# sbelharbi/feature-vs-text-compound-emotion

Measured on AMD Instinct MI355X. Metric: training clips/sec (32-frame tri-modal clip), higher is better.
Workload: dtype bf16x3 (split hi/lo bf16 operands, 3 MFMAs per product, fp32 accumulate; <= 2^-15 relative per product)

## Files before the change

### feature_vs_text_compound_emotion_amd/csrc/conv_b3.h

```cpp
#pragma once
#include "conv_common.h"

namespace cer {

typedef __bf16 bf16x8 __attribute__((ext_vector_type(8)));
typedef unsigned int u32x4 __attribute__((ext_vector_type(4)));
typedef __attribute__((address_space(3))) void *lds_ptr_t;

__device__ __forceinline__ bf16x8 as_bf16x8(const u32x4 v) { return __builtin_bit_cast(bf16x8, v); }


typedef float f32x4 __attribute__((ext_vector_type(4)));
__device__ __forceinline__ int swz16(int q) { return (0x78 >> (2 * q)) & 3; }

int conv_b3_patch_launch(int tile, const ConvArgs &a, hipStream_t st);
bool conv_b3_patch_ok(const ConvArgs &a);
bool conv_b3_win_ok(const ConvArgs &a);
int conv_b3_s2d_launch(int tile, const ConvArgs &a, hipStream_t st);
bool conv_b3_s2d_ok(const ConvArgs &a);

}
```

### feature_vs_text_compound_emotion_amd/csrc/conv_b3.hip

```cpp
#include "conv_b3.h"

namespace cer {

template <int BM, int BN, int WP, int WC, int NW = 4, int STAGES = 2>
__global__ __launch_bounds__(NW * 64, NW == 4 ? 2 : 1) void conv_b3_dma16_kernel(ConvArgs p) {
    static_assert(WP * WC == NW && BM % (16 * NW) == 0 && BN % (16 * NW) == 0, "1-KiB pieces are dealt round-robin to the waves");
    constexpr int BKT = 32, ROWB = BKT * 2;
    constexpr int XP = BM / (16 * NW), WQ = BN / (16 * NW);
    constexpr int PX = BM * ROWB, PW = BN * ROWB;
    constexpr int BUF = 2 * PX + 2 * PW;
    constexpr int NDMA = 2 * XP + 2 * WQ;
    static_assert(STAGES == 2 || STAGES == 3, "ring depth");
    constexpr int TP = BM / (16 * WP), TC = BN / (16 * WC);
    constexpr unsigned OOB = 0x80000000u;
    extern __shared__ __attribute__((aligned(16))) uint16_t smem_b3[];
    unsigned char *smem = reinterpret_cast<unsigned char *>(smem_b3);

    const int tid = threadIdx.x, lane = tid & 63;
    const int wave = __builtin_amdgcn_readfirstlane(tid >> 6);
    const int wp = wave % WP, wc = wave / WP;
    const int kg = lane >> 4, l15 = lane & 15;

    const int nwg = p.tiles_m * p.tiles_n;
    int bid = blockIdx.x;
// ... 247 lines not shown
                    const int m = m0 + (wp * TP + b) * 16 + l15;
                    const float v = (m < p.M) ? acc[a][b][r] : 0.f;
                    s1 += v;
                    s2 += v * v;
                });
#pragma unroll
                for (int o = 8; o > 0; o >>= 1) {
                    s1 += __shfl_xor(s1, o);
                    s2 += __shfl_xor(s2, o);
                }
                if (l15 == 0) {
                    const int ci = (wc * TC + a) * 16 + 4 * kg + r;
                    red[(wp * 2 + 0) * BN + ci] = s1;
                    red[(wp * 2 + 1) * BN + ci] = s2;
                }
            });
        });
        __syncthreads();
        if (tid < BN && c0 + tid < p.Cout) {
            float s1 = 0.f, s2 = 0.f;
#pragma unroll
            for (int w = 0; w < WP; ++w) {
                s1 += red[(w * 2 + 0) * BN + tid];
                s2 += red[(w * 2 + 1) * BN + tid];
            }
            p.stats[((size_t)tile_m * 2 + 0) * p.Cout + c0 + tid] = s1;
            p.stats[((size_t)tile_m * 2 + 1) * p.Cout + c0 + tid] = s2;
        }
    }
}

__global__ void split_bf16_kernel(const float4 *__restrict__ x, const float *__restrict__ scale,
                                  const float *__restrict__ shift, ushort4 *__restrict__ hi, ushort4 *__restrict__ lo,
                                  size_t n4, int C4) {
    size_t i = (size_t)blockIdx.x * blockDim.x + threadIdx.x;
    if (i >= n4) return;
    float4 v = x[i];
    if (scale) {
        const int c = (int)(i % C4) * 4;
        const float4 s = *reinterpret_cast<const float4 *>(scale + c), t = *reinterpret_cast<const float4 *>(shift + c);
        v = make_float4(v.x * s.x + t.x, v.y * s.y + t.y, v.z * s.z + t.z, v.w * s.w + t.w);
    }
    ushort4 h, l;
    split_bf16(v.x, h.x, l.x); split_bf16(v.y, h.y, l.y);
    split_bf16(v.z, h.z, l.z); split_bf16(v.w, h.w, l.w);
    hi[i] = h;
    lo[i] = l;
}

template <int BM, int BN, int WP, int WC, int NW = 4, int STAGES = 2>
static int launch_b3_dma16(const ConvArgs &a, hipStream_t st) {
    if ((long long)BN * a.Kpad * 2 >= (1ll << 31))
        return cer_set_error(CER_ERR_UNSUPPORTED, "conv2d (bf16x3, LDS-DMA): weight panel exceeds 31-bit offsets");
    const size_t lds = (size_t)STAGES * (2 * BM + 2 * BN) * 64;
    auto k = conv_b3_dma16_kernel<BM, BN, WP, WC, NW, STAGES>;
    if (lds > 64 * 1024) CER_HIP_CHECK(hipFuncSetAttribute((const void *)k, hipFuncAttributeMaxDynamicSharedMemorySize, (int)lds));
    CER_LAUNCH(k, dim3(a.tiles_m * a.tiles_n, 1, a.split_k), dim3(NW * 64), lds, st, a);
    CER_HIP_CHECK(hipGetLastError());
    return CER_OK;
}

static bool b3_patch_geometry(const cer_conv_desc *d) {
    return d->KH == 3 && d->KW == 3 && d->stride == 1 && d->dil_h == 1 && d->dil_w == 1 && d->pad_t == 1 && d->pad_l == 1 &&
           d->Ho == d->H && d->Wo == d->W && (d->H & 15) == 0 && (d->W & 15) == 0 && (d->Cin & 31) == 0 && d->split_k <= 1;
}

static bool b3_win_geometry(const cer_conv_desc *d) {
    return d->KH == 3 && d->KW == 3 && d->stride == 1 && d->dil_h == 1 && d->dil_w == 1 && d->pad_t == 1 && d->pad_l == 1 &&
           d->Ho == d->H && d->Wo == d->W && d->H >= 2 && d->W >= 2 && d->W <= 86 && (d->Cin & 31) == 0 && d->split_k <= 1;
}

int conv_b3_tile_dims(const cer_conv_desc *d, int &bm, int &bn, int &bk) {
    int tile = d->tile;
    const long long M = (long long)d->N * d->Ho * d->Wo;
    const int Cout = d->Cout;
    if (d->x_s2d) {
        if (tile == 0) tile = Cout > 64 ? 52 : 51;
        else if (tile != 51 && tile != 52) return 0;
    } else if (tile == 51 || tile == 52) {
        return 0;
    }
    if (tile == 0) {
        const long long t128 = (M + 127) / 128 * ((Cout + 127) / 128), t256 = (M + 255) / 256;
        if (b3_patch_geometry(d) && Cout <= 64 && t256 >= 512) tile = 59;
        else if (b3_patch_geometry(d) && Cout >= 128 && t256 * ((Cout + 127) / 128) >= 512) tile = 58;
        else if (b3_win_geometry(d) && t256 >= 64) tile = Cout > 64 ? 56 : 53;
        else if (Cout <= 64) tile = t256 >= 512 ? 48 : 42;
        else if (t128 >= 512) tile = 41;
        else tile = Cout >= 128 ? 44 : 45;
    }
    bk = 32;
    switch (tile) {
        case 41: bm = 128; bn = 128; break;
        case 42: bm = 128; bn = 64; break;
        case 44: bm = 64; bn = 128; break;
        case 45: bm = 64; bn = 64; break;
        case 48: bm = 256; bn = 64; break;
        case 59: bm = 256; bn = 64; break;
        case 58: bm = 256; bn = 128; break;
        case 53: bm = 256; bn = 64; break;
        case 56: bm = 256; bn = 128; break;
        case 51: bm = 256; bn = 64; break;
        case 52: bm = 256; bn = 128; break;
        default: return 0;
    }
    return tile;
}

int conv_b3_launch(int tile, const ConvArgs &a, hipStream_t st) {
    switch (tile) {
        case 41: return launch_b3_dma16<128, 128, 2, 2>(a, st);
        case 42: return launch_b3_dma16<128, 64, 2, 2>(a, st);
        case 44: return launch_b3_dma16<64, 128, 1, 4>(a, st);
        case 45: return launch_b3_dma16<64, 64, 2, 2>(a, st);
        case 48: return launch_b3_dma16<256, 64, 4, 1>(a, st);
        case 53: case 56: case 58: case 59: return conv_b3_patch_launch(tile, a, st);
        case 51: case 52: return conv_b3_s2d_launch(tile, a, st);
        default: return cer_set_error(CER_ERR_INVALID_ARG, "conv2d (bf16x3): unknown tile id");
    }
}

}

using namespace cer;

extern "C" int cer_conv2d_b3_tile(const cer_conv_desc *d) {
    if (!d || d->N <= 0 || d->Ho <= 0 || d->Wo <= 0 || d->Cout <= 0) return 0;
    int bm, bn, bk;
    return conv_b3_tile_dims(d, bm, bn, bk);
}

extern "C" int cer_split_bf16(const float *x, const float *scale, const float *shift, int C, uint16_t *hi, uint16_t *lo,
                              size_t n, void *stream) {
    if (!x || !hi || !lo || n == 0 || (n & 3)) return cer_set_error(CER_ERR_INVALID_ARG, "split_bf16: n must be a positive multiple of 4");
    if ((scale == nullptr) != (shift == nullptr) || (scale && (C <= 0 || (C & 3) || n % C)))
        return cer_set_error(CER_ERR_INVALID_ARG, "split_bf16: the per-channel affine needs scale, shift and C % 4 == 0 dividing n");
    CER_LAUNCH(split_bf16_kernel, dim3(cer_blocks(n / 4, 256)), dim3(256), 0, (hipStream_t)stream, (const float4 *)x, scale,
               shift, (ushort4 *)hi, (ushort4 *)lo, n / 4, scale ? C / 4 : 1);
    CER_HIP_CHECK(hipGetLastError());
    return CER_OK;
}
```

### feature_vs_text_compound_emotion_amd/csrc/conv_b3_patch.hip

```cpp
#include "conv_b3.h"

namespace cer {

constexpr unsigned long long B3_PATCH_F_TABLE = 0xaaa00a00ull;
__device__ __forceinline__ int b3_patch_f(int wx) { return (int)((B3_PATCH_F_TABLE >> (2 * wx)) & 3ull); }

struct B3PatchGeo { FastDiv tiles_n, pxn, pyn; };

template <int BN, int WP, int WC, bool SINGLE>
__global__ __launch_bounds__(WP * WC * 64, 2) void conv_b3_patch_kernel(ConvArgs p, B3PatchGeo geo) {
    constexpr int NW = WP * WC, NT = NW * 64;
    constexpr int PH = 16, PWD = 16, WW = 18, WROWS = 18 * 18;
    constexpr int XPP = (WROWS + 15) / 16;
    constexpr int XPW = (XPP + NW - 1) / NW;
    constexpr int XPL = XPP * 1024, XBYTES = 2 * XPL;
    constexpr int WPL = BN * 64, WSLICE = 2 * WPL;
    constexpr int WPIECES = 2 * BN / 16;
    static_assert(WPIECES % NW == 0, "weight-slice pieces are dealt round-robin to the waves");
    constexpr int WQ = WPIECES / NW;
    constexpr int TP = PH / WP, TC = BN / (16 * WC);
    static_assert(PH % WP == 0 && (SINGLE || XPW <= 9) && TP >= 2 && TC % 2 == 0, "geometry");
    static_assert(SINGLE ? WC == 1 : (WP == 4 && WC == 2 && (BN / 16) % 4 == 0), "ping-pong: waves w and w + 4 share a SIMD and split the couts");
    constexpr int WOFF = (SINGLE ? 1 : 2) * XBYTES, SINK = WOFF + 3 * WSLICE;
    constexpr unsigned OOB = 0x80000000u;
    extern __shared__ __attribute__((aligned(16))) uint16_t smem_b3p[];
    unsigned char *smem = reinterpret_cast<unsigned char *>(smem_b3p);

    const int tid = threadIdx.x, lane = tid & 63;
    const int wave = __builtin_amdgcn_readfirstlane(tid >> 6);
    const int wp = wave % WP, wc = wave / WP;
    const int kg = lane >> 4, l15 = lane & 15;

    const int nwg = p.tiles_m * p.tiles_n;
    int bid = blockIdx.x;
    {
        const int q = nwg >> 3, r = nwg & 7, xcd = bid & 7, idx = bid >> 3;
        bid = (xcd < r ? xcd * (q + 1) : r * (q + 1) + (xcd - r) * q) + idx;
    }
    const int patch = (int)fdiv((unsigned)bid, geo.tiles_n), tile_n = bid - patch * p.tiles_n;
    const int prw = (int)fdiv((unsigned)patch, geo.pxn), px = patch - prw * (int)geo.pxn.d;
    const int n = (int)fdiv((unsigned)prw, geo.pyn), py = prw - n * (int)geo.pyn.d;
    const int c0 = tile_n * BN;
    const int cin_steps = p.cin_steps;

    const int prow = lane >> 2, slot = lane & 3;
    unsigned x_off[XPW];
    bool x_real[XPW];
    {
        const int iy0 = py * PH - 1, ix0 = px * PWD - 1, pitch = p.x_ld * 2;
#pragma unroll
        for (int i = 0; i < XPW; ++i) {
            const int q = wave + NW * i;
            const int row = q * 16 + prow;
            const int wy = row / WW, wx = row - wy * WW;
            const int iy = iy0 + wy, ix = ix0 + wx;
            const bool inb = q < XPP && row < WROWS && (unsigned)iy < (unsigned)p.H && (unsigned)ix < (unsigned)p.W;
            x_real[i] = q < XPP;
            x_off[i] = inb ? (unsigned)((iy * p.W + ix) * pitch) + (unsigned)((slot ^ b3_patch_f(wx)) << 4) : OOB;
        }
    }
    unsigned w_off[WQ];
    int w_plane[WQ], w_dst[WQ];
#pragma unroll
    for (int i = 0; i < WQ; ++i) {
        const int j = SINGLE ? wave + NW * i : (wave & 3) + 4 * i;
        constexpr int PPL = SINGLE ? BN / 16 : BN / 32;
        w_plane[i] = j / PPL;
        const int pc = (SINGLE ? 0 : (wave >> 2) * PPL) + j % PPL;
        const int row = pc * 16 + prow;
        const int grow = row / (TC * 16) * (TC * 16) + epi_cout_of_row(row % (TC * 16));
        w_dst[i] = w_plane[i] * WPL + pc * 1024;
        w_off[i] = c0 + grow < p.Cout ? (unsigned)(grow * p.Kpad * 2) + (unsigned)((slot ^ swz16((row >> 2) & 3)) << 4) : OOB;
    }
    const size_t img = (size_t)n * p.H * p.W * p.x_ld * 2;
    const char *xh = reinterpret_cast<const char *>(p.x_hi) + img, *xl = reinterpret_cast<const char *>(p.x_lo) + img;
    const size_t wpan = (size_t)c0 * p.Kpad * 2;
    const char *wh = reinterpret_cast<const char *>(p.w_hi) + wpan, *wl = reinterpret_cast<const char *>(p.w_lo) + wpan;

    auto issue_x = [&](int i, int cc) {
        const bool real = x_real[i] && cc < cin_steps;
        const __amdgpu_buffer_rsrc_t rh = __builtin_amdgcn_make_buffer_rsrc(const_cast<char *>(xh) + (size_t)cc * 64, 0, (int)OOB, 0x00020000);
        const __amdgpu_buffer_rsrc_t rl = __builtin_amdgcn_make_buffer_rsrc(const_cast<char *>(xl) + (size_t)cc * 64, 0, (int)OOB, 0x00020000);
        unsigned char *dst = real ? smem + (SINGLE ? 0 : (cc & 1) * XBYTES) + (wave + NW * i) * 1024 : smem + SINK;
        const int vo = (int)(real ? x_off[i] : OOB);
        __builtin_amdgcn_raw_ptr_buffer_load_lds(rh, (lds_ptr_t)dst, 16, vo, 0, 0, 0);
        __builtin_amdgcn_raw_ptr_buffer_load_lds(rl, (lds_ptr_t)(real ? dst + XPL : dst), 16, vo, 0, 0, 0);
    };
    auto issue_w = [&](int cc, int tap, int ring) {
        const bool real = cc < cin_steps;
        const size_t koff = ((size_t)tap * p.Cin + (size_t)cc * 32) * 2;
// ... 591 lines not shown
```

### feature_vs_text_compound_emotion_amd/csrc/conv_igemm.hip

```cpp
#include <hip/hip_runtime.h>
#include <stdint.h>

#include "cer_internal.h"
#include "conv_common.h"

namespace cer {

template <int BM, int BN, int WP, int WC, bool VEC, int VAR, int BKT>
__global__ __launch_bounds__(WP * WC * 64, 3) void conv_igemm_kernel(ConvArgs p) {
    constexpr int NT = WP * WC * 64;
    constexpr int CH = BKT / 4;
    constexpr int RPP = NT / CH;
    constexpr int PIT = BKT + 4;
    constexpr int NG = BKT / 8;
    constexpr bool PRIO = (VAR & 1) != 0, SINGLE = (VAR & 2) != 0, BLKPRIO = (VAR & 4) != 0;
    constexpr bool ABL_NOSTAGE = (VAR & 8) != 0;
    constexpr bool ABL_NOBAR = (VAR & 16) != 0;
    constexpr int NBUF = SINGLE ? 1 : 2;
    constexpr int TP = BM / (32 * WP);
    constexpr int TC = BN / (32 * WC);
    constexpr int XR = BM / RPP;
    constexpr int WR = BN / RPP;
    extern __shared__ __attribute__((aligned(16))) float smem[];
    float *Xs = smem;
// ... 316 lines not shown
        if (t.bn > 64 && d->Cout <= 64) continue;
        const long long blocks = (long long)((M + t.bm - 1) / t.bm) * ((d->Cout + t.bn - 1) / t.bn) * d->split_k;
        const long long slots = 256ll * t.per_cu;
        const long long rounds = (blocks + slots - 1) / slots;
        const float frac = (float)(blocks - (rounds - 1) * slots) / (float)slots;
        const float eff_rounds = (float)(rounds - 1) + (frac < 0.5f ? 0.5f + frac * 0.5f : (frac < 1.f ? 0.75f + frac * 0.25f : 1.f));
        const float time = eff_rounds * (float)(t.bm * t.bn) * (float)t.per_cu / t.rate;
        if (time < best_t) { best_t = time; best = t.id; }
    }
    return best;
}

static void tile_dims(int tile, int &bm, int &bn) {
    switch (tile) {
        case 1: bm = 128; bn = 128; break;
        case 2: bm = 128; bn = 64; break;
        case 4: bm = 64; bn = 128; break;
        default: bm = 64; bn = 64; break;
    }
}

template <int VAR>
static int launch_shape(int shape, const ConvArgs &a, bool vec, hipStream_t st) {
    switch (shape) {
        case 1: return launch_cfg<128, 128, 2, 2, VAR>(a, vec, st);
        case 2: return launch_cfg<128, 64, 2, 2, VAR>(a, vec, st);
        case 4: return launch_cfg<64, 128, 1, 4, VAR>(a, vec, st);
        case 5: return launch_cfg<64, 64, 2, 2, VAR>(a, vec, st);
        default: return cer_set_error(CER_ERR_INVALID_ARG, "conv2d_fwd: unknown tile id");
    }
}

}

using namespace cer;

extern "C" int cer_conv_kpad(int KH, int KW, int Cin) {
    int K = KH * KW * Cin;
    return (K + BK - 1) / BK * BK;
}

static int validate_desc(const cer_conv_desc *d) {
    if (!d) return cer_set_error(CER_ERR_INVALID_ARG, "conv desc is NULL");
    if (d->N <= 0 || d->H <= 0 || d->W <= 0 || d->Cin <= 0 || d->Ho <= 0 || d->Wo <= 0 || d->Cout <= 0 ||
        d->KH <= 0 || d->KW <= 0 || d->stride <= 0 || d->dil_h <= 0 || d->dil_w <= 0 || d->split_k < 1)
        return cer_set_error(CER_ERR_INVALID_ARG, "conv desc: non-positive dimension");
    if ((long long)d->N * d->Ho * d->Wo >= (1ll << 31) || (long long)d->N * d->H * d->W >= (1ll << 31))
        return cer_set_error(CER_ERR_UNSUPPORTED, "conv desc: more than 2^31 pixels");
    if (d->x_nchw && (d->Cin % 32) == 0)
        return cer_set_error(CER_ERR_UNSUPPORTED, "conv desc: NCHW input only on the small-Cin path");
    return CER_OK;
}

namespace cer {
int conv_b3_tile_dims(const cer_conv_desc *d, int &bm, int &bn, int &bk);
int conv_n16_tile_dims(const cer_conv_desc *d, int &bm, int &bn, int &bk);
}

extern "C" int cer_conv2d_stats_tiles(const cer_conv_desc *d, int kernel_family) {
    if (!d || d->N <= 0 || d->Ho <= 0 || d->Wo <= 0) return 0;
    const int M = d->N * d->Ho * d->Wo;
    int bm, bn, bk;
    if (kernel_family == 2) {
        if (!conv_n16_tile_dims(d, bm, bn, bk)) return 0;
    } else if (kernel_family == 1) {
        const int t = conv_b3_tile_dims(d, bm, bn, bk);
        if (!t) return 0;
        if (t == 6) return 2 * ((M + bm - 1) / bm);
    } else {
        tile_dims(pick_tile(d, M), bm, bn);
    }
    return (M + bm - 1) / bm;
}

extern "C" size_t cer_conv2d_workspace_bytes(const cer_conv_desc *d) {
    if (!d || d->split_k <= 1) return 0;
    return (size_t)d->split_k * d->N * d->Ho * d->Wo * d->Cout * sizeof(float);
}

namespace cer {
int conv_b3_launch(int tile, const ConvArgs &a, hipStream_t st);
int conv_n16_launch(int tile, const ConvArgs &a, hipStream_t st);
bool conv_n16_p64_ok(const ConvArgs &a);
}

extern "C" int cer_conv2d_run(const cer_conv_desc *d, const cer_conv_io *io, void *workspace, size_t workspace_bytes,
                              void *stream) {
    int rc = validate_desc(d);
    if (rc) return rc;
    if (!io) return cer_set_error(CER_ERR_INVALID_ARG, "conv2d: io block is NULL");
    if (d->storage != CER_STORE_NONE && d->storage != CER_STORE_BF16 && d->storage != CER_STORE_F16)
        return cer_set_error(CER_ERR_INVALID_ARG, "conv2d: unknown storage type");
    const bool narrow = d->storage != CER_STORE_NONE;
    const bool n16 = narrow && io->x_hi != nullptr;
    const bool b3 = !narrow && io->x_hi != nullptr;
    if (narrow && (io->x_lo || io->w_lo || io->y_lo || io->res_lo || io->y2_hi || io->y2_lo))
        return cer_set_error(CER_ERR_INVALID_ARG, "conv2d (narrow): 16-bit tensors are single planes (every *_lo and y2 pointer must be NULL)");
    if (n16) {
        if (!io->w_hi) return cer_set_error(CER_ERR_INVALID_ARG, "conv2d (narrow): x_hi and w_hi must both be given");
        if (io->in_scale || io->mask || io->aux || d->x_nchw)
            return cer_set_error(CER_ERR_UNSUPPORTED, "conv2d (narrow): no input affine / mask / aux / NCHW input");
    } else if (b3) {
        if (!io->x_lo || !io->w_hi || !io->w_lo)
            return cer_set_error(CER_ERR_INVALID_ARG, "conv2d (bf16x3): x_hi, x_lo, w_hi, w_lo must all be given");
        if (io->in_scale || io->mask || io->aux || d->x_nchw)
            return cer_set_error(CER_ERR_UNSUPPORTED, "conv2d (bf16x3): no input affine / mask / aux / NCHW input");
    } else if (!io->x || !io->w) {
        return cer_set_error(CER_ERR_INVALID_ARG, "conv2d: x and w must be non-NULL");
    }
    if (!io->y && !io->y_hi && !io->y2_hi) return cer_set_error(CER_ERR_INVALID_ARG, "conv2d: no output tensor");
    if ((io->in_scale == nullptr) != (io->in_shift == nullptr))
        return cer_set_error(CER_ERR_INVALID_ARG, "conv2d: in_scale and in_shift go together");
    if (!narrow && ((io->y_hi == nullptr) != (io->y_lo == nullptr) || (io->res_hi == nullptr) != (io->res_lo == nullptr) ||
                    (io->y2_hi == nullptr) != (io->y2_lo == nullptr) || (io->y2_hi && (!io->s2 || !io->t2))))
        return cer_set_error(CER_ERR_INVALID_ARG, "conv2d: split tensors need both planes (and s2/t2 for the second output)");
    if (io->residual && io->res_hi) return cer_set_error(CER_ERR_INVALID_ARG, "conv2d: give the residual as fp32 OR split");
    if (d->act1 == CER_ACT_PRELU && !io->alpha) return cer_set_error(CER_ERR_INVALID_ARG, "conv2d: PReLU needs alpha");
    const bool has_res = io->residual || io->res_hi;
    if (has_res && (d->res_stride <= 0 || d->Hr <= 0 || d->Wr <= 0 || (d->Ho - 1) * d->res_stride >= d->Hr ||
                    (d->Wo - 1) * d->res_stride >= d->Wr))
        return cer_set_error(CER_ERR_INVALID_ARG, "conv2d: residual geometry out of range");
    if (io->stats && d->split_k > 1)
        return cer_set_error(CER_ERR_UNSUPPORTED, "conv2d: batch statistics are not available with split-K");
    if ((io->y_hi || io->y2_hi || io->res_hi) && (d->Cout & 3))
        return cer_set_error(CER_ERR_UNSUPPORTED, "conv2d: split outputs / residual need Cout % 4 == 0");
    ConvArgs a{};
    a.x = io->x; a.w = io->w; a.in_scale = io->in_scale; a.in_shift = io->in_shift; a.bias = io->bias; a.alpha = io->alpha;
    a.res = io->residual; a.mask = io->mask; a.y = io->y; a.aux = io->aux; a.stats = io->stats;
    a.x_hi = io->x_hi; a.x_lo = io->x_lo; a.w_hi = io->w_hi; a.w_lo = io->w_lo;
    a.res_hi = io->res_hi; a.res_lo = io->res_lo; a.y_hi = io->y_hi; a.y_lo = io->y_lo;
    a.s2 = io->s2; a.t2 = io->t2; a.y2_hi = io->y2_hi; a.y2_lo = io->y2_lo;
    a.bias9 = io->bias9;
    a.narrow = d->storage;
    if (io->bias9 && (io->bias || d->stride != 1 || d->Ho != d->H || d->Wo != d->W || d->H < 2 || d->W < 2 || d->split_k > 1))
        return cer_set_error(CER_ERR_INVALID_ARG, "conv2d: bias9 replaces bias and needs a stride-1 same conv on >= 2x2 images without split-K");
    if (d->x_s2d || d->y_s2d) {
        if (!b3 && !n16) return cer_set_error(CER_ERR_UNSUPPORTED, "conv2d: space-to-depth tensors exist in the bf16x3 and narrow modes only");
        if (d->x_s2d && d->x_ld > 0) return cer_set_error(CER_ERR_INVALID_ARG, "conv2d: x_s2d fixes the input pitch (x_ld must be 0)");
        if (d->y_s2d && ((d->Ho | d->Wo) & 1 || io->y || io->y2_hi || has_res || io->mask || io->aux || d->y_ld > 0 || !io->y_hi))
            return cer_set_error(CER_ERR_INVALID_ARG, "conv2d: y_s2d needs even Ho / Wo and a plain 16-bit output (no fp32 / second "
                                                      "output, residual, mask, aux or y_ld)");
    }
    a.x_s2d = d->x_s2d != 0; a.y_s2d = d->y_s2d != 0;
    a.x_ld = d->x_s2d ? 4 * d->Cin : (d->x_ld > 0 ? d->x_ld : d->Cin);
    a.y_ld = d->y_ld > 0 ? d->y_ld : d->Cout;
    if (a.x_ld < d->Cin || a.y_ld < d->Cout || ((d->Cin % 32) == 0 && (a.x_ld & 3) != 0))
        return cer_set_error(CER_ERR_INVALID_ARG, "conv2d: x_ld/y_ld smaller than the channel count or x_ld % 4 != 0");
    if (d->x_nchw && d->x_ld > 0) return cer_set_error(CER_ERR_INVALID_ARG, "conv2d: x_ld is meaningless for NCHW input");
    a.N = d->N; a.H = d->H; a.W = d->W; a.Cin = d->Cin; a.Ho = d->Ho; a.Wo = d->Wo; a.Cout = d->Cout;
    a.KH = d->KH; a.KW = d->KW; a.stride = d->stride; a.dil_h = d->dil_h; a.dil_w = d->dil_w;
    a.pad_t = d->pad_t; a.pad_l = d->pad_l; a.x_nchw = d->x_nchw;
    a.res_stride = d->res_stride; a.Hr = d->Hr; a.Wr = d->Wr; a.act1 = d->act1; a.act2 = d->act2;
    a.slope = d->slope;
    a.Kpad = cer_conv_kpad(d->KH, d->KW, d->Cin);
    a.M = d->N * d->Ho * d->Wo;
    const bool vec = (d->Cin % 32) == 0;
    int tile, bm, bn, bk, esz;
    if (n16) {
        tile = conv_n16_tile_dims(d, bm, bn, bk);
        if (!tile) return cer_set_error(CER_ERR_INVALID_ARG, "conv2d (narrow): unknown tile id (space-to-depth input: 81 / 82 only)");
        if (d->y_s2d && tile != 71 && tile != 72 && tile != 78 && tile != 73 && tile != 76 && tile != 77 && tile != 79)
            return cer_set_error(CER_ERR_UNSUPPORTED, "conv2d (narrow): y_s2d is written by the window / patch kernels only "
                                                      "(cer_conv2d_n16_tile(desc) in {71, 72, 73, 76, 77, 78, 79})");
        if (d->Cin % bk != 0 || (a.x_ld & 7))
            return cer_set_error(CER_ERR_UNSUPPORTED, "conv2d (narrow): Cin must be a multiple of 64 and x_ld of 8");
        esz = 2;
    } else if (b3) {
        tile = conv_b3_tile_dims(d, bm, bn, bk);
        if (!tile) return cer_set_error(CER_ERR_INVALID_ARG, "conv2d (bf16x3): unknown tile id (space-to-depth input: 51 / 52 only)");
        if (d->y_s2d && tile != 53 && tile != 56 && tile != 58 && tile != 59)
            return cer_set_error(CER_ERR_UNSUPPORTED, "conv2d (bf16x3): y_s2d is written by the window / patch kernels only "
                                                      "(cer_conv2d_b3_tile(desc) in {53, 56, 58, 59})");
        if (d->Cin % bk != 0 || (a.x_ld & 7))
            return cer_set_error(CER_ERR_UNSUPPORTED, "conv2d (bf16x3): Cin must be a multiple of the K step and x_ld of 8");
        esz = 2;
    } else {
        tile = pick_tile(d, a.M);
        if (tile != 1 && tile != 2 && tile != 4 && tile != 5) return cer_set_error(CER_ERR_INVALID_ARG, "conv2d: unknown tile id");
        bk = 32;
        tile_dims(tile, bm, bn);
        esz = 4;
    }
    a.cin_steps = (vec || b3 || n16) ? d->Cin / bk : 1;
    a.steps = a.Kpad / bk;
    a.split_k = d->split_k > a.steps ? a.steps : d->split_k;
    a.steps_per_split = (a.steps + a.split_k - 1) / a.split_k;
    a.split_k = (a.steps + a.steps_per_split - 1) / a.steps_per_split;
    a.tiles_m = (a.M + bm - 1) / bm;
    a.tiles_n = (a.Cout + bn - 1) / bn;
    if (vec || b3 || n16) {
        if (d->KH * d->KW > 32) return cer_set_error(CER_ERR_UNSUPPORTED, "conv2d: more than 32 filter taps");
        if (d->Wo > d->W / d->stride + 1 ||
            (long long)d->H * d->W < (long long)(d->Ho - 1) * d->stride * d->W + (long long)(d->Wo - 1) * d->stride)
            return cer_set_error(CER_ERR_UNSUPPORTED, "conv2d: the output grid outruns the input (Ho/Wo too large for H/W and stride)");
        const long long span_px = (long long)bm * d->stride * d->stride + 2ll * d->H * d->W + (long long)d->W * d->stride + 2;
        if (span_px * a.x_ld * esz >= (1ll << 31) || (long long)bn * a.Kpad * esz >= (1ll << 32))
            return cer_set_error(CER_ERR_UNSUPPORTED, "conv2d: tile footprint exceeds 32-bit staging offsets");
    }
    hipStream_t st = (hipStream_t)stream;
    ConvArgs fin = a;
    if (a.split_k > 1) {
        size_t need = (size_t)a.split_k * a.M * a.Cout * sizeof(float);
        if (!workspace || workspace_bytes < need) return cer_set_error(CER_ERR_WORKSPACE, "conv2d: split-K workspace too small");
        a.y = (float *)workspace;
    }
    if (n16) {
        if (tile == 79 && d->tile == 0 && !conv_n16_p64_ok(a)) tile = 71;
        rc = conv_n16_launch(tile, a, st);
    } else if (b3) {
        rc = conv_b3_launch(tile, a, st);
    } else {
        rc = launch_shape<2>(tile, a, vec, st);
    }
    if (rc) return rc;
    if (a.split_k > 1) {
        fin.split_k = a.split_k;
        size_t n = (size_t)a.M * ((a.Cout + 3) / 4);
        CER_LAUNCH(splitk_reduce_kernel, dim3((unsigned)((n + 255) / 256)), dim3(256), 0, st, fin, (const float *)workspace);
        CER_HIP_CHECK(hipGetLastError());
    }
    return CER_OK;
}

extern "C" int cer_conv2d_fwd(const cer_conv_desc *d, const float *x, const float *w, const float *in_scale,
                              const float *in_shift, const float *bias, const float *alpha, const float *residual,
                              const float *mask, float *y, float *aux, float *stats, void *workspace,
                              size_t workspace_bytes, void *stream) {
    if (!x || !w || !y) return cer_set_error(CER_ERR_INVALID_ARG, "conv2d_fwd: x, w, y must be non-NULL");
    cer_conv_io io{};
    io.x = x; io.w = w; io.in_scale = in_scale; io.in_shift = in_shift; io.bias = bias; io.alpha = alpha;
    io.residual = residual; io.mask = mask; io.y = y; io.aux = aux; io.stats = stats;
    return cer_conv2d_run(d, &io, workspace, workspace_bytes, stream);
}
```

### feature_vs_text_compound_emotion_amd/ops.py

```python
import ctypes
import os

import torch

from . import _lib
from ._lib import (ACT_GELU, ACT_LEAKY, ACT_NONE, ACT_PRELU, ACT_RELU, STORE_BF16, STORE_F16, STORE_NONE, ConvDesc,
                   ConvIO, check, current_stream, ptr)

LEAKY_SLOPE = 0.01


def _dev_f32(t, name, contiguous=True):
    if t is None:
        return
    if not (t.is_cuda and t.dtype == torch.float32 and (t.is_contiguous() or not contiguous)):
        raise ValueError(f"{name}: expected a contiguous float32 tensor on the GPU, got "
                         f"{t.dtype} {t.device} contiguous={t.is_contiguous()}")


def _rows(t, name):
    if not (t.is_cuda and t.dtype == torch.float32 and t.dim() == 2 and t.stride(1) == 1):
        raise ValueError(f"{name}: expected a 2-D float32 GPU tensor with unit column stride")
    return t.shape[0], t.shape[1], (t.stride(0) if t.shape[0] > 1 else max(t.stride(0), t.shape[1]))

# ... 193 lines not shown
            io.res_hi, io.res_lo = residual.hi.data_ptr(), residual.lo.data_ptr()
        else:
            _dev_f32(residual, "residual")
            io.residual = residual.data_ptr()
    res = {}
    dev = x.hi.device
    if out_f32:
        res["y"] = torch.empty((n, ho, wo, cout), device=dev, dtype=torch.float32)
        io.y = res["y"].data_ptr()
    if out_split:
        res["split"] = Split.empty((n, ho // 2, wo // 2, 4 * cout) if y_s2d else (n, ho, wo, cout), dev)
        io.y_hi, io.y_lo = res["split"].hi.data_ptr(), res["split"].lo.data_ptr()
    if next_affine is not None:
        s2, t2 = next_affine
        _dev_f32(s2, "s2")
        _dev_f32(t2, "t2")
        res["next"] = Split.empty((n, ho, wo, cout), dev)
        io.s2, io.t2 = s2.data_ptr(), t2.data_ptr()
        io.y2_hi, io.y2_lo = res["next"].hi.data_ptr(), res["next"].lo.data_ptr()
    if want_stats:
        res["stats"] = torch.empty((lib.cer_conv2d_stats_tiles(ctypes.byref(d), 1), 2, cout), device=dev,
                                   dtype=torch.float32)
        io.stats = res["stats"].data_ptr()
    ws_bytes = lib.cer_conv2d_workspace_bytes(ctypes.byref(d))
    ws = torch.empty((ws_bytes // 4,), device=dev, dtype=torch.float32) if ws_bytes else None
    if CONV_TRACE is not None:
        e0, e1 = torch.cuda.Event(enable_timing=True), torch.cuda.Event(enable_timing=True)
        e0.record()
    check(lib.cer_conv2d_run(ctypes.byref(d), ctypes.byref(io), ptr(ws), ws_bytes, current_stream()), "cer_conv2d_run")
    if CONV_TRACE is not None:
        e1.record()
        nout = n * ho * wo * cout
        nbytes = 4.0 * n * h * wd * cin + 4.0 * nout * (int(out_f32) + int(out_split) + int(next_affine is not None)) + \
            4.0 * cout * cin * kh * kw + (4.0 * nout if residual is not None else 0.0)
        CONV_TRACE.append((lib.cer_conv2d_b3_tile(ctypes.byref(d)), 2.0 * n * ho * wo * cout * cin * kh * kw, e0, e1, nbytes))
    return res


def stem_conv(x, w, scale=None, shift=None, alpha=None, out=None, want_stats=False):
    _dev_f32(x, "x")
    _dev_f32(w, "w")
    for t, nme in ((scale, "scale"), (shift, "shift"), (alpha, "alpha")):
        _dev_f32(t, nme)
    n, c, h, wd = x.shape
    if c != 3 or w.shape[0] != 64:
        raise ValueError("stem_conv is the 3 -> 64 input layer")
    lib = _lib.load()
    stats = _empty((lib.cer_stem_conv3x3_stats_rows(n, h), 2, 64), x) if (want_stats or out is None) else None
    res, y, hi, lo, storage = {}, None, None, None, STORE_NONE
    if out == "f32":
        res["y"] = y = torch.empty((n, h, wd, 64), device=x.device, dtype=torch.float32)
    elif out == "split":
        res["split"] = Split.empty((n, h, wd, 64), x.device)
        hi, lo = res["split"].hi, res["split"].lo
    elif out is not None:
        storage = storage_of(out)
        res["n16"] = hi = torch.empty((n, h, wd, 64), device=x.device, dtype=out)
    check(lib.cer_stem_conv3x3(ptr(x), ptr(w), w.shape[1], ptr(scale), ptr(shift), ptr(alpha), ptr(y), ptr(hi), ptr(lo), storage,
                               ptr(stats), n, h, wd, current_stream()), "cer_stem_conv3x3")
    if out is None:
        return stats
    if want_stats:
        res["stats"] = stats
    return res


def _tile_desc(n, h, w, cin, cout, kh, kw, stride, pad, x_s2d):
    d = ConvDesc()
    d.N, d.H, d.W, d.Cin, d.Cout = n, h, w, cin, cout
    d.Ho, d.Wo = (h + 2 * pad[0] - kh) // stride + 1, (w + 2 * pad[1] - kw) // stride + 1
    d.KH, d.KW, d.stride, d.dil_h, d.dil_w, d.pad_t, d.pad_l = kh, kw, stride, 1, 1, pad[0], pad[1]
    d.split_k, d.x_s2d = 1, int(x_s2d)
    return d


def conv2d_b3_tile(n, h, w, cin, cout, kh, kw, stride, pad, x_s2d=False):
    return _lib.load().cer_conv2d_b3_tile(ctypes.byref(_tile_desc(n, h, w, cin, cout, kh, kw, stride, pad, x_s2d)))


def conv2d_n16_tile(n, h, w, cin, cout, kh, kw, stride, pad, x_s2d=False):
    return _lib.load().cer_conv2d_n16_tile(ctypes.byref(_tile_desc(n, h, w, cin, cout, kh, kw, stride, pad, x_s2d)))


S2D_PRODUCER_TILES = (53, 56, 58, 59)
S2D_PRODUCER_TILES_N16 = (71, 72, 73, 76, 77, 78, 79)


def s2d_k_order(cin, device, chunk=32):
    order = (ctypes.c_int32 * (9 * cin))()
    check(_lib.load().cer_conv_s2d_k_order(cin, chunk, order), "cer_conv_s2d_k_order")
    return torch.tensor(list(order), dtype=torch.long, device=device)


def pack_s2d_weight(w, cin, chunk=None):
    if isinstance(w, Split):
        idx = s2d_k_order(cin, w.hi.device, chunk or 32)
        return Split(w.hi.index_select(1, idx).contiguous(), w.lo.index_select(1, idx).contiguous())
    return w.index_select(1, s2d_k_order(cin, w.device, chunk or 64)).contiguous()


def space_to_depth(x):
    if isinstance(x, Split):
        return Split(space_to_depth(x.hi), space_to_depth(x.lo))
    return torch.cat([x[:, 1::2, 1::2], x[:, 1::2, 0::2], x[:, 0::2, 1::2], x[:, 0::2, 0::2]], dim=3).contiguous()


def storage_of(dtype):
    if dtype == torch.bfloat16:
        return STORE_BF16
    if dtype == torch.float16:
        return STORE_F16
    raise ValueError(f"narrow storage is torch.bfloat16 or torch.float16, got {dtype}")


def _dev_n16(t, name, dtype=None):
    if t is None:
        return
    if not (t.is_cuda and t.dtype in (torch.bfloat16, torch.float16) and t.is_contiguous()) or (dtype is not None and t.dtype != dtype):
        raise ValueError(f"{name}: expected a contiguous {dtype or 'bfloat16/float16'} GPU tensor, got {t.dtype} {t.device}")


def to_n16(x, dtype, scale=None, shift=None):
    _dev_f32(x, "x")
    _dev_f32(scale, "scale")
    _dev_f32(shift, "shift")
    out = torch.empty(x.shape, device=x.device, dtype=dtype)
    c = x.shape[-1] if scale is not None else 0
    check(_lib.load().cer_to_n16(ptr(x), ptr(scale), ptr(shift), c, ptr(out), x.numel(), storage_of(dtype), current_stream()),
          "cer_to_n16")
    return out


def from_n16(x):
    _dev_n16(x, "x")
    out = torch.empty(x.shape, device=x.device, dtype=torch.float32)
    check(_lib.load().cer_from_n16(ptr(x), ptr(out), x.numel(), storage_of(x.dtype), current_stream()), "cer_from_n16")
    return out


def conv2d_n16(x, w, kh, kw, *, stride=1, dil=(1, 1), pad=(0, 0), out_hw=None, bias=None, alpha=None, residual=None,
               res_stride=1, act1=ACT_NONE, act2=ACT_NONE, slope=LEAKY_SLOPE, split_k=1, tile=0, out_f32=False,
               out_n16=True, want_stats=False, bias9=None, x_s2d=False, y_s2d=False):
    lib = _lib.load()
    _dev_n16(x, "x")
    _dev_n16(w, "w", x.dtype)
    _dev_f32(bias, "bias")
    _dev_f32(alpha, "alpha")
    n, h, wd, cin = x.shape
    if x_s2d:
        if cin % 4:
            raise ValueError("a space-to-depth input has 4 * Cin channels")
        h, wd, cin = 2 * h, 2 * wd, cin // 4
    cout = w.shape[0]
    if w.shape[1] != conv_kpad(kh, kw, cin):
        raise ValueError(f"packed weight has K={w.shape[1]}, expected {conv_kpad(kh, kw, cin)}")
    if out_hw is None:
        ho = (h + 2 * pad[0] - dil[0] * (kh - 1) - 1) // stride + 1
        wo = (wd + 2 * pad[1] - dil[1] * (kw - 1) - 1) // stride + 1
    else:
        ho, wo = out_hw
    d = ConvDesc()
    d.N, d.H, d.W, d.Cin, d.Ho, d.Wo, d.Cout = n, h, wd, cin, ho, wo, cout
    d.KH, d.KW, d.stride, d.dil_h, d.dil_w, d.pad_t, d.pad_l = kh, kw, stride, dil[0], dil[1], pad[0], pad[1]
    d.res_stride, d.Hr, d.Wr = res_stride, 0, 0
    d.act1, d.act2, d.slope, d.split_k, d.tile = act1, act2, slope, split_k, tile
    d.storage = storage_of(x.dtype)
    d.x_s2d, d.y_s2d = int(x_s2d), int(y_s2d)
# ... 739 lines not shown
```

Before: 59.68.

## Add persistent bf16x3 patch conv kernel for Cin=64 3x3 layers

Adds a persistent 3x3 conv kernel for bf16x3 inputs with Cin=64, selected as tile 69 for large images. It keeps all nine taps of the weight slice resident in LDS and runs two wave groups in ping-pong, so one group does MFMA while the other runs the epilogue and prefetches the next input window. Patches are spread over XCDs. The goal is to hide epilogue and load latency and avoid reloading weights per tile. It falls back to tiles 58/59 when the epilogue mode is not supported. The grid is sized to the CU count, which adds load-balance risk.

New measurement: 60.20, median of 6. Within noise of the previous version (+0.9%).

```diff
diff --git a/feature_vs_text_compound_emotion_amd/csrc/conv_b3.h b/feature_vs_text_compound_emotion_amd/csrc/conv_b3.h
--- a/feature_vs_text_compound_emotion_amd/csrc/conv_b3.h
+++ b/feature_vs_text_compound_emotion_amd/csrc/conv_b3.h
@@ -13,10 +13,17 @@
 typedef float f32x4 __attribute__((ext_vector_type(4)));
 __device__ __forceinline__ int swz16(int q) { return (0x78 >> (2 * q)) & 3; }
 
+constexpr unsigned long long B3_PATCH_F_TABLE = 0xaaa00a00ull;
+__device__ __forceinline__ int b3_patch_f(int wx) { return (int)((B3_PATCH_F_TABLE >> (2 * wx)) & 3ull); }
+
+struct B3PatchGeo { FastDiv tiles_n, pxn, pyn; };
+
 int conv_b3_patch_launch(int tile, const ConvArgs &a, hipStream_t st);
 bool conv_b3_patch_ok(const ConvArgs &a);
 bool conv_b3_win_ok(const ConvArgs &a);
 int conv_b3_s2d_launch(int tile, const ConvArgs &a, hipStream_t st);
 bool conv_b3_s2d_ok(const ConvArgs &a);
+int conv_b3_p64_launch(const ConvArgs &a, hipStream_t st);
+bool conv_b3_p64_ok(const ConvArgs &a);
 
 }
diff --git a/feature_vs_text_compound_emotion_amd/csrc/conv_b3.hip b/feature_vs_text_compound_emotion_amd/csrc/conv_b3.hip
--- a/feature_vs_text_compound_emotion_amd/csrc/conv_b3.hip
+++ b/feature_vs_text_compound_emotion_amd/csrc/conv_b3.hip
@@ -353,7 +353,8 @@
     }
     if (tile == 0) {
         const long long t128 = (M + 127) / 128 * ((Cout + 127) / 128), t256 = (M + 255) / 256;
-        if (b3_patch_geometry(d) && Cout <= 64 && t256 >= 512) tile = 59;
+        if (b3_patch_geometry(d) && d->Cin == 64 && (Cout & 63) == 0 && Cout <= 256 && t256 >= 2048) tile = 69;
+        else if (b3_patch_geometry(d) && Cout <= 64 && t256 >= 512) tile = 59;
         else if (b3_patch_geometry(d) && Cout >= 128 && t256 * ((Cout + 127) / 128) >= 512) tile = 58;
         else if (b3_win_geometry(d) && t256 >= 64) tile = Cout > 64 ? 56 : 53;
         else if (Cout <= 64) tile = t256 >= 512 ? 48 : 42;
@@ -369,6 +370,7 @@
         case 48: bm = 256; bn = 64; break;
         case 59: bm = 256; bn = 64; break;
         case 58: bm = 256; bn = 128; break;
+        case 69: bm = 256; bn = 64; break;
         case 53: bm = 256; bn = 64; break;
         case 56: bm = 256; bn = 128; break;
         case 51: bm = 256; bn = 64; break;
@@ -386,6 +388,7 @@
         case 45: return launch_b3_dma16<64, 64, 2, 2>(a, st);
         case 48: return launch_b3_dma16<256, 64, 4, 1>(a, st);
         case 53: case 56: case 58: case 59: return conv_b3_patch_launch(tile, a, st);
+        case 69: return conv_b3_p64_launch(a, st);
         case 51: case 52: return conv_b3_s2d_launch(tile, a, st);
         default: return cer_set_error(CER_ERR_INVALID_ARG, "conv2d (bf16x3): unknown tile id");
     }
diff --git a/feature_vs_text_compound_emotion_amd/csrc/conv_b3_p64.hip b/feature_vs_text_compound_emotion_amd/csrc/conv_b3_p64.hip
--- /dev/null
+++ b/feature_vs_text_compound_emotion_amd/csrc/conv_b3_p64.hip
@@ -0,0 +1,290 @@
+#include "conv_b3.h"
+
+namespace cer {
+
+namespace {
+constexpr int BP_BN = 32, BP_XPP = 21, BP_XPL = BP_XPP * 1024, BP_XBYTES = 2 * BP_XPL;
+constexpr int BP_WPL = BP_BN * 64, BP_WSLICE = 2 * BP_WPL, BP_WOFF = 2 * BP_XBYTES, BP_STOFF = BP_WOFF + 18 * BP_WSLICE;
+constexpr int BP_LDS = BP_STOFF + 2 * 4 * 2 * BP_BN * 4;
+}
+
+__global__ __launch_bounds__(512, 2) void conv_b3_p64_kernel(ConvArgs p, B3PatchGeo geo) {
+    constexpr int BN = BP_BN, NWG = 4, WP = 4, TP = 4, TC = 2, PH = 16, PWD = 16, WW = 18, WROWS = 18 * 18;
+    constexpr int XPP = BP_XPP, XPW = (XPP + NWG - 1) / NWG, XPL = BP_XPL, XBYTES = BP_XBYTES;
+    constexpr int WPL = BP_WPL, WSLICE = BP_WSLICE, WOFF = BP_WOFF, STOFF = BP_STOFF;
+    constexpr unsigned OOB = 0x80000000u;
+    extern __shared__ __attribute__((aligned(16))) uint16_t smem_b3p64[];
+    unsigned char *smem = reinterpret_cast<unsigned char *>(smem_b3p64);
+
+    const int tid = threadIdx.x, lane = tid & 63;
+    const int wave = __builtin_amdgcn_readfirstlane(tid >> 6);
+    const int grp = wave >> 2, wp = wave & 3;
+    const int kg = lane >> 4, l15 = lane & 15;
+    const int prow = lane >> 2, slot = lane & 3;
+
+    const int xcd = blockIdx.x & 7, kblk = blockIdx.x >> 3, nbx = gridDim.x >> 3;
+    const int kq = (int)fdiv((unsigned)kblk, geo.tiles_n), tile_n = kblk - kq * p.tiles_n;
+    const int pstride = nbx / p.tiles_n;
+    const int q8 = p.tiles_m >> 3, r8 = p.tiles_m & 7;
+    const int plo = xcd * q8 + (xcd < r8 ? xcd : r8), pcnt = q8 + (xcd < r8 ? 1 : 0);
+    const int c0 = tile_n * BN;
+    if (kq >= pcnt) return;
+    const int nblk = (pcnt - kq + pstride - 1) / pstride;
+    const int nmine = (nblk - grp + 1) >> 1;
+    const int nunits = 2 * nmine;
+
+#pragma unroll
+    for (int i = 0; i < 9; ++i) {
+        const int q = wave + 8 * i, s = q >> 2, pl = (q >> 1) & 1, half = q & 1;
+        const int cc = s / 9, tap = s - 9 * cc;
+        const int row = half * 16 + prow;
+        const int grow = epi_cout_of_row(row);
+        const char *base = reinterpret_cast<const char *>(pl ? p.w_lo : p.w_hi) + (size_t)c0 * p.Kpad * 2 + ((size_t)tap * p.Cin + cc * 32) * 2;
+        const __amdgpu_buffer_rsrc_t rw = __builtin_amdgcn_make_buffer_rsrc(const_cast<char *>(base), 0, (int)OOB, 0x00020000);
+        const unsigned off = c0 + grow < p.Cout ? (unsigned)(grow * p.Kpad * 2) + (unsigned)((slot ^ swz16((row >> 2) & 3)) << 4) : OOB;
+        __builtin_amdgcn_raw_ptr_buffer_load_lds(rw, (lds_ptr_t)(smem + WOFF + s * WSLICE + pl * WPL + half * 1024), 16, (int)off, 0, 0, 0);
+    }
+
+    const int pitch = p.x_ld * 2;
+    int wyx[XPW];
+    unsigned xrel[XPW];
+#pragma unroll
+    for (int i = 0; i < XPW; ++i) {
+        const int qp = wp + NWG * i;
+        const int row = qp * 16 + prow;
+        const int wy = row / WW, wx = row - wy * WW;
+        const bool live = qp < XPP && row < WROWS;
+        wyx[i] = live ? wy * 32 + wx : -1;
+        xrel[i] = live ? (unsigned)((wy * p.W + wx) * pitch) + (unsigned)((slot ^ b3_patch_f(wx)) << 4) : OOB;
+    }
+    struct Patch { int n, py, px, id; };
+    auto patch_of = [&](int jj) __attribute__((always_inline)) {
+        Patch t;
+        t.id = plo + kq + (2 * jj + grp) * pstride;
+        const int prw = (int)fdiv((unsigned)t.id, geo.pxn);
+        t.px = t.id - prw * (int)geo.pxn.d;
+        t.n = (int)fdiv((unsigned)prw, geo.pyn);
+        t.py = prw - t.n * (int)geo.pyn.d;
+        return t;
+    };
+    auto issue_window = [&](const Patch &t, int cc) __attribute__((always_inline)) {
+        const int iy0 = t.py * PH - 1, ix0 = t.px * PWD - 1;
+        const int base = (iy0 * p.W + ix0) * pitch;
+        const bool interior = t.py > 0 && t.py < (int)geo.pyn.d - 1 && t.px > 0 && t.px < (int)geo.pxn.d - 1;
+        const size_t img = (size_t)t.n * p.H * p.W * p.x_ld * 2 + (size_t)cc * 64;
+        const __amdgpu_buffer_rsrc_t rh = __builtin_amdgcn_make_buffer_rsrc(
+            const_cast<char *>(reinterpret_cast<const char *>(p.x_hi) + img), 0, (int)OOB, 0x00020000);
+        const __amdgpu_buffer_rsrc_t rl = __builtin_amdgcn_make_buffer_rsrc(
+            const_cast<char *>(reinterpret_cast<const char *>(p.x_lo) + img), 0, (int)OOB, 0x00020000);
+#pragma unroll
+        for (int i = 0; i < XPW; ++i) {
+            if (wp + NWG * i < XPP) {
+                bool inb = wyx[i] >= 0;
+                if (!interior) {
+                    const int iy = iy0 + (wyx[i] >> 5), ix = ix0 + (wyx[i] & 31);
+                    inb = inb && (unsigned)iy < (unsigned)p.H && (unsigned)ix < (unsigned)p.W;
+                }
+                const int off = inb ? base + (int)xrel[i] : (int)OOB;
+                unsigned char *dst = smem + grp * XBYTES + (wp + NWG * i) * 1024;
+                __builtin_amdgcn_raw_ptr_buffer_load_lds(rh, (lds_ptr_t)dst, 16, off, 0, 0, 0);
+                __builtin_amdgcn_raw_ptr_buffer_load_lds(rl, (lds_ptr_t)(dst + XPL), 16, off, 0, 0, 0);
+            }
+        }
+    };
+
+    const int arow = l15 * 64 + ((kg ^ swz16((l15 >> 2) & 3)) << 4);
+    int bcol[3];
+#pragma unroll
+    for (int kw = 0; kw < 3; ++kw) bcol[kw] = (wp * WW + kw + l15) * 64 + ((kg ^ b3_patch_f(kw + l15)) << 4);
+    const unsigned char *Xb = smem + grp * XBYTES;
+    const int emode = epi_mode(p);
+
+    f32x4 acc[TC][TP];
+
+    auto k_phase = [&](int cc) __attribute__((always_inline)) {
+        const unsigned char *Wc = smem + WOFF + cc * 9 * WSLICE + arow;
+        if (cc == 0) {
+#pragma unroll
+            for (int a = 0; a < TC; ++a)
+#pragma unroll
+                for (int b = 0; b < TP; ++b)
+#pragma unroll
+                    for (int r = 0; r < 4; ++r) acc[a][b][r] = 0.f;
+        }
+        u32x4 ah[2][TC], al[2][TC], bh[2][TP], bl[2][TP];
+        auto read_tap = [&](auto Tt, int set) {
+            constexpr int tap = decltype(Tt)::v, kh = tap / 3, kw = tap % 3;
+#pragma unroll
+            for (int a = 0; a < TC; ++a) {
+                ah[set][a] = *reinterpret_cast<const u32x4 *>(Wc + tap * WSLICE + a * 16 * 64);
+                al[set][a] = *reinterpret_cast<const u32x4 *>(Wc + tap * WSLICE + WPL + a * 16 * 64);
+            }
+#pragma unroll
+            for (int b = 0; b < TP; ++b) {
+                bh[set][b] = *reinterpret_cast<const u32x4 *>(Xb + kh * (WW * 64) + bcol[kw] + b * WP * WW * 64);
+                bl[set][b] = *reinterpret_cast<const u32x4 *>(Xb + XPL + kh * (WW * 64) + bcol[kw] + b * WP * WW * 64);
+            }
+        };
+        read_tap(IdxC<0>{}, 0);
+        __builtin_amdgcn_sched_group_barrier(0x100, 12, 0);
+        static_for<9>([&](auto Tt) {
+            constexpr int tap = decltype(Tt)::v, set = tap & 1;
+            if constexpr (tap < 8) read_tap(IdxC<tap + 1>{}, set ^ 1);
+#pragma unroll
+            for (int a = 0; a < TC; ++a)
+#pragma unroll
+                for (int b = 0; b < TP; ++b)
+                    acc[a][b] = __builtin_amdgcn_mfma_f32_16x16x32_bf16(as_bf16x8(al[set][a]), as_bf16x8(bh[set][b]), acc[a][b], 0, 0, 0);
+#pragma unroll
+            for (int a = 0; a < TC; ++a)
+#pragma unroll
+                for (int b = 0; b < TP; ++b)
+                    acc[a][b] = __builtin_amdgcn_mfma_f32_16x16x32_bf16(as_bf16x8(ah[set][a]), as_bf16x8(bl[set][b]), acc[a][b], 0, 0, 0);
+#pragma unroll
+            for (int a = 0; a < TC; ++a)
+#pragma unroll
+                for (int b = 0; b < TP; ++b)
+                    acc[a][b] = __builtin_amdgcn_mfma_f32_16x16x32_bf16(as_bf16x8(ah[set][a]), as_bf16x8(bh[set][b]), acc[a][b], 0, 0, 0);
+            if constexpr (tap < 8) {
+                __builtin_amdgcn_sched_group_barrier(0x100, 12, 0);
+                __builtin_amdgcn_sched_group_barrier(0x008, 24, 0);
+            }
+        });
+    };
+
+    auto walk = [&](auto MODE_, auto STATS_) __attribute__((always_inline)) {
+        constexpr int MODE = decltype(MODE_)::v;
+        constexpr bool STATS = decltype(STATS_)::v;
+        constexpr int NST = 2 * TP;
+        float aa[8], bb[8];
+        epi_direct_consts<MODE>(p, c0 + kg * 8, aa, bb);
+        float *part = reinterpret_cast<float *>(smem + STOFF) + grp * (4 * 2 * BN);
+        auto flush_stats = [&](const Patch &t) __attribute__((always_inline)) {
+            const int st = lane >> 5, c = lane & 31;
+            float s = 0.f;
+#pragma unroll
+            for (int w = 0; w < 4; ++w) s += part[(w * 2 + st) * BN + c];
+            p.stats[((size_t)t.id * 2 + st) * p.Cout + c0 + c] = s;
+        };
+        auto e_phase = [&](int u) __attribute__((always_inline)) {
+            const int jj = u >> 1;
+            const Patch t = patch_of(jj);
+            if ((u & 1) == 0) {
+                issue_window(t, 1);
+                __builtin_amdgcn_sched_barrier(0);
+                if constexpr (STATS) {
+                    if (jj > 0 && wp == 0) {
+                        flush_stats(patch_of(jj - 1));
+                        __builtin_amdgcn_sched_barrier(0);
+                        asm volatile("s_waitcnt vmcnt(1)" ::: "memory");
+                        return;
+                    }
+                }
+                asm volatile("s_waitcnt vmcnt(0)" ::: "memory");
+                return;
+            }
+            if (jj + 1 < nmine) issue_window(patch_of(jj + 1), 0);
+            __builtin_amdgcn_sched_barrier(0);
+            float s1[8], s2[8];
+#pragma unroll
+            for (int e = 0; e < 8; ++e) s1[e] = s2[e] = 0.f;
+            const int c = c0 + kg * 8;
+            static_for<TP>([&](auto B) {
+                constexpr int b = decltype(B)::v;
+                const int gy = t.py * PH + b * WP + wp, gx = t.px * PWD + l15;
+                const int m = (t.n * p.H + gy) * p.W + gx;
+                const float v[8] = {acc[0][b][0], acc[0][b][1], acc[0][b][2], acc[0][b][3],
+                                    acc[1][b][0], acc[1][b][1], acc[1][b][2], acc[1][b][3]};
+                if constexpr (STATS) {
+#pragma unroll
+                    for (int e = 0; e < 8; ++e) {
+                        s1[e] += v[e];
+                        s2[e] += v[e] * v[e];
+                    }
+                }
+                const size_t orow = (size_t)(p.y_s2d ? s2d_row(m, gy, gx, p.W) : m);
+                if constexpr (MODE == EPI_B9_PRELU_SPLIT) {
+                    const int ry = gy == 0 ? 0 : (gy == p.H - 1 ? 2 : 1), rx = gx == 0 ? 0 : (gx == p.W - 1 ? 2 : 1);
+                    const int cs = 3 * ry + rx;
+                    if (__ballot(cs != 4) != 0ull) epi_direct8<MODE, CER_STORE_BF16, true>(p, aa, bb, orow, c, cs, v);
+                    else epi_direct8<MODE, CER_STORE_BF16, false>(p, aa, bb, orow, c, 4, v);
+                } else {
+                    epi_direct8<MODE, CER_STORE_BF16, false>(p, aa, bb, orow, c, 4, v);
+                }
+            });
+            if constexpr (STATS) {
+#pragma unroll
+                for (int e = 0; e < 8; ++e) {
+                    s1[e] = row16_sum(s1[e]);
+                    s2[e] = row16_sum(s2[e]);
+                }
+                if (l15 == 0) {
+                    float *d1 = part + (wp * 2 + 0) * BN + kg * 8, *d2 = d1 + BN;
+                    *reinterpret_cast<float4 *>(d1) = make_float4(s1[0], s1[1], s1[2], s1[3]);
+                    *reinterpret_cast<float4 *>(d1 + 4) = make_float4(s1[4], s1[5], s1[6], s1[7]);
+                    *reinterpret_cast<float4 *>(d2) = make_float4(s2[0], s2[1], s2[2], s2[3]);
+                    *reinterpret_cast<float4 *>(d2 + 4) = make_float4(s2[4], s2[5], s2[6], s2[7]);
+                }
+            }
+            __builtin_amdgcn_sched_barrier(0);
+            asm volatile("s_waitcnt vmcnt(%0)" ::"n"(NST) : "memory");
+        };
+
+        if (nunits > 0) issue_window(patch_of(0), 0);
+        asm volatile("s_waitcnt vmcnt(0)" ::: "memory");
+        __builtin_amdgcn_s_barrier();
+        const int nph = 4 * ((nblk + 1) >> 1) + 1;
+        for (int ph = 0; ph < nph; ++ph) {
+            const bool kph = ((ph ^ grp) & 1) == 0;
+            if (kph) {
+                const int u = (ph - grp) >> 1;
+                if (ph >= grp && u < nunits) k_phase(u & 1);
+            } else {
+                const int u = (ph - 1 - grp) >> 1;
+                if (ph - 1 >= grp && u < nunits) e_phase(u);
+            }
+            asm volatile("s_waitcnt lgkmcnt(0)" ::: "memory");
+            __builtin_amdgcn_sched_barrier(0);
+            __builtin_amdgcn_s_barrier();
+            __builtin_amdgcn_sched_barrier(0);
+        }
+        if constexpr (STATS) {
+            if (nmine > 0 && wp == 0) flush_stats(patch_of(nmine - 1));
+        }
+    };
+    if (emode == EPI_RAW_F32) {
+        if (p.stats) walk(IdxC<EPI_RAW_F32>{}, IdxC<1>{});
+        else walk(IdxC<EPI_RAW_F32>{}, IdxC<0>{});
+    } else if (emode == EPI_B9_PRELU_SPLIT) {
+        walk(IdxC<EPI_B9_PRELU_SPLIT>{}, IdxC<0>{});
+    }
+}
+
+bool conv_b3_p64_ok(const ConvArgs &a) {
+    if (!conv_b3_patch_ok(a) || a.Cin != 64 || a.x_s2d || a.narrow || (a.Cout & 63) || a.Kpad != 9 * 64) return false;
+    const int mode = epi_mode(a);
+    return mode == EPI_RAW_F32 || (mode == EPI_B9_PRELU_SPLIT && !a.stats);
+}
+
+int conv_b3_p64_launch(const ConvArgs &a, hipStream_t st) {
+    if (!conv_b3_p64_ok(a))
+        return cer_set_error(CER_ERR_UNSUPPORTED, "conv2d (bf16x3, persistent patch kernel): needs a 3x3 / stride 1 / pad 1 conv on "
+                                                   "images whose height and width are multiples of 16, Cin == 64, Cout % 64 == 0 "
+                                                   "and one of the specialised epilogues (bias9 + PReLU -> split, raw -> fp32)");
+    int dev = 0, cus = 0;
+    CER_HIP_CHECK(hipGetDevice(&dev));
+    CER_HIP_CHECK(hipDeviceGetAttribute(&cus, hipDeviceAttributeMultiprocessorCount, dev));
+    ConvArgs b = a;
+    b.tiles_n = a.Cout / BP_BN;
+    const int unit = 8 * b.tiles_n;
+    const int grid = cus / unit * unit;
+    if (grid <= 0) return cer_set_error(CER_ERR_UNSUPPORTED, "conv2d (bf16x3, persistent patch kernel): fewer CUs than 8 x cout tiles");
+    const B3PatchGeo geo{make_fastdiv((unsigned)b.tiles_n), make_fastdiv((unsigned)(a.W / 16)), make_fastdiv((unsigned)(a.H / 16))};
+    auto k = conv_b3_p64_kernel;
+    CER_HIP_CHECK(hipFuncSetAttribute((const void *)k, hipFuncAttributeMaxDynamicSharedMemorySize, BP_LDS));
+    CER_LAUNCH(k, dim3(grid), dim3(512), BP_LDS, st, b, geo);
+    CER_HIP_CHECK(hipGetLastError());
+    return CER_OK;
+}
+
+}
diff --git a/feature_vs_text_compound_emotion_amd/csrc/conv_b3_patch.hip b/feature_vs_text_compound_emotion_amd/csrc/conv_b3_patch.hip
--- a/feature_vs_text_compound_emotion_amd/csrc/conv_b3_patch.hip
+++ b/feature_vs_text_compound_emotion_amd/csrc/conv_b3_patch.hip
@@ -1,11 +1,6 @@
 #include "conv_b3.h"
 
 namespace cer {
-
-constexpr unsigned long long B3_PATCH_F_TABLE = 0xaaa00a00ull;
-__device__ __forceinline__ int b3_patch_f(int wx) { return (int)((B3_PATCH_F_TABLE >> (2 * wx)) & 3ull); }
-
-struct B3PatchGeo { FastDiv tiles_n, pxn, pyn; };
 
 template <int BN, int WP, int WC, bool SINGLE>
 __global__ __launch_bounds__(WP * WC * 64, 2) void conv_b3_patch_kernel(ConvArgs p, B3PatchGeo geo) {
diff --git a/feature_vs_text_compound_emotion_amd/csrc/conv_igemm.hip b/feature_vs_text_compound_emotion_amd/csrc/conv_igemm.hip
--- a/feature_vs_text_compound_emotion_amd/csrc/conv_igemm.hip
+++ b/feature_vs_text_compound_emotion_amd/csrc/conv_igemm.hip
@@ -422,6 +422,7 @@
 int conv_b3_launch(int tile, const ConvArgs &a, hipStream_t st);
 int conv_n16_launch(int tile, const ConvArgs &a, hipStream_t st);
 bool conv_n16_p64_ok(const ConvArgs &a);
+bool conv_b3_p64_ok(const ConvArgs &a);
 }
 
 extern "C" int cer_conv2d_run(const cer_conv_desc *d, const cer_conv_io *io, void *workspace, size_t workspace_bytes,
@@ -508,9 +509,9 @@
     } else if (b3) {
         tile = conv_b3_tile_dims(d, bm, bn, bk);
         if (!tile) return cer_set_error(CER_ERR_INVALID_ARG, "conv2d (bf16x3): unknown tile id (space-to-depth input: 51 / 52 only)");
-        if (d->y_s2d && tile != 53 && tile != 56 && tile != 58 && tile != 59)
+        if (d->y_s2d && tile != 53 && tile != 56 && tile != 58 && tile != 59 && tile != 69)
             return cer_set_error(CER_ERR_UNSUPPORTED, "conv2d (bf16x3): y_s2d is written by the window / patch kernels only "
-                                                      "(cer_conv2d_b3_tile(desc) in {53, 56, 58, 59})");
+                                                      "(cer_conv2d_b3_tile(desc) in {53, 56, 58, 59, 69})");
         if (d->Cin % bk != 0 || (a.x_ld & 7))
             return cer_set_error(CER_ERR_UNSUPPORTED, "conv2d (bf16x3): Cin must be a multiple of the K step and x_ld of 8");
         esz = 2;
@@ -548,6 +549,10 @@
         if (tile == 79 && d->tile == 0 && !conv_n16_p64_ok(a)) tile = 71;
         rc = conv_n16_launch(tile, a, st);
     } else if (b3) {
+        if (tile == 69 && d->tile == 0 && !conv_b3_p64_ok(a)) {
+            tile = a.Cout <= 64 ? 59 : 58;
+            a.tiles_n = (a.Cout + (tile == 59 ? 63 : 127)) / (tile == 59 ? 64 : 128);
+        }
         rc = conv_b3_launch(tile, a, st);
     } else {
         rc = launch_shape<2>(tile, a, vec, st);
diff --git a/feature_vs_text_compound_emotion_amd/ops.py b/feature_vs_text_compound_emotion_amd/ops.py
--- a/feature_vs_text_compound_emotion_amd/ops.py
+++ b/feature_vs_text_compound_emotion_amd/ops.py
@@ -299,7 +299,7 @@
     return _lib.load().cer_conv2d_n16_tile(ctypes.byref(_tile_desc(n, h, w, cin, cout, kh, kw, stride, pad, x_s2d)))
 
 
-S2D_PRODUCER_TILES = (53, 56, 58, 59)
+S2D_PRODUCER_TILES = (53, 56, 58, 59, 69)
 S2D_PRODUCER_TILES_N16 = (71, 72, 73, 76, 77, 78, 79)
 
 
```
